# intel/neural-compressor

Hardware: AMD Instinct MI355X
Metric: llama2_7b_gptq_int4_g128_quantize_wall_clock (lower is better)
Workload: dtype bf16

## Files before the change

neural_compressor_amd/csrc/gptq.hip:

```cpp
#include <math.h>

#include <algorithm>
#include <type_traits>

#include "common.hpp"
#include "gptq_common.hpp"

namespace {

typedef __attribute__((ext_vector_type(16))) float f32x16;

template <int DT>
__global__ void gptq_prepare_weight_kernel(const void* __restrict__ w, float* __restrict__ out,
                                           const uint8_t* __restrict__ dead, int64_t N, int64_t K) {
  const int64_t total = N * K;
  for (int64_t i = blockIdx.x * (int64_t)blockDim.x + threadIdx.x; i < total;
       i += (int64_t)gridDim.x * blockDim.x) {
    const int64_t k = i % K;
    out[i] = (dead && dead[k]) ? 0.f : load_as_f32<DT>(w, i);
  }
}
template <int DT>
__global__ __launch_bounds__(256) void gptq_prepare_weight_vec_kernel(const void* __restrict__ w, float* __restrict__ out,
                                                                      const uint8_t* __restrict__ dead, int64_t N, int64_t K) {
  const int64_t k8 = K >> 3, total = N * k8;
  for (int64_t i = blockIdx.x * (int64_t)blockDim.x + threadIdx.x; i < total; i += (int64_t)gridDim.x * blockDim.x) {
    const int64_t n = i / k8, c = (i - n * k8) << 3, base = n * K + c;
    float v[8];
    if constexpr (DT == INC_F32) {
      const float4 a = reinterpret_cast<const float4*>(static_cast<const float*>(w) + base)[0];
      const float4 b = reinterpret_cast<const float4*>(static_cast<const float*>(w) + base)[1];
      v[0] = a.x; v[1] = a.y; v[2] = a.z; v[3] = a.w; v[4] = b.x; v[5] = b.y; v[6] = b.z; v[7] = b.w;
    } else {
      const uint4 q = *reinterpret_cast<const uint4*>(static_cast<const uint16_t*>(w) + base);
      const uint32_t u[4] = {q.x, q.y, q.z, q.w};
#pragma unroll
      for (int e = 0; e < 4; ++e) {
        if constexpr (DT == INC_BF16) {
          v[2 * e] = bf16_bits_to_f32((uint16_t)(u[e] & 0xffffu));
          v[2 * e + 1] = bf16_bits_to_f32((uint16_t)(u[e] >> 16));
        } else {
          v[2 * e] = f16_bits_to_f32((uint16_t)(u[e] & 0xffffu));
          v[2 * e + 1] = f16_bits_to_f32((uint16_t)(u[e] >> 16));
        }
      }
    }
    if (dead) {
      const uint2 d = *reinterpret_cast<const uint2*>(dead + c);
#pragma unroll
      for (int e = 0; e < 8; ++e)
        if (((e < 4 ? d.x : d.y) >> (8 * (e & 3))) & 0xffu) v[e] = 0.f;
    }
    reinterpret_cast<float4*>(out + base)[0] = make_float4(v[0], v[1], v[2], v[3]);
    reinterpret_cast<float4*>(out + base)[1] = make_float4(v[4], v[5], v[6], v[7]);
  }
}

constexpr int QROWS = 64;
constexpr int QPITCH = QB + 1;

#pragma clang fp contract(off)
template <int QDT>
__global__ __launch_bounds__(64) void gptq_quant_block_kernel(
    const float* __restrict__ w, const float* __restrict__ Hinv, const float* __restrict__ scale,
    const float* __restrict__ zero, uint8_t* __restrict__ codes, void* __restrict__ q_out,
    float* __restrict__ err, int64_t N, int64_t K, int64_t G, int64_t i1, int count, int gs, float maxq) {
  extern __shared__ __attribute__((aligned(16))) char smem_raw[];
  float* hs = reinterpret_cast<float*>(smem_raw);
  float* stage = hs + QB * QB;
  uint8_t* cst = reinterpret_cast<uint8_t*>(stage + QROWS * QPITCH);
  constexpr int CP = QB + 4;
  const int lane = threadIdx.x;
  const int64_t n0 = (int64_t)blockIdx.x * QROWS;
  const int64_t row = n0 + lane;

  for (int idx = lane; idx < QB * QB; idx += 64) {
    const int r = idx >> 7, c = idx & 127;
    hs[idx] = (r < count && c < count) ? Hinv[(i1 + r) * K + i1 + c] : (r == c ? 1.f : 0.f);
  }
  for (int idx = lane; idx < QROWS * QB; idx += 64) {
    const int r = idx >> 7, c = idx & 127;
    stage[r * QPITCH + c] = (n0 + r < N && c < count) ? w[(n0 + r) * K + i1 + c] : 0.f;
  }
  __syncthreads();
  float wr[QB];
#pragma unroll
  for (int j = 0; j < QB; ++j) wr[j] = stage[lane * QPITCH + j];
  __syncthreads();

  const int64_t srow = (row < N ? row : N - 1) * G;
  int g = gs > 0 ? (int)(i1 / gs) : 0;
  int nb = gs > 0 ? (int)(((int64_t)(g + 1)) * gs - i1) : (1 << 30);
  float s = scale[srow + g], z = zero[srow + g];
#pragma unroll
  for (int i = 0; i < QB; ++i) {
    if (i < count) {
      if (i == nb) {
        ++g;
        nb += gs;
        s = scale[srow + g];
        z = zero[srow + g];
      }
      const float d = hs[i * QB + i];
      const float x = wr[i];
      float t = rintf(x / s) + z;
      t = fminf(fmaxf(t, 0.f), maxq);
      const float q = s * (t - z);
      const float e = (x - q) / d;
      cst[lane * CP + i] = (uint8_t)t;
      stage[lane * QPITCH + i] = e;
      wr[i] = q;
#pragma unroll
      for (int j = i + 1; j < QB; ++j) {
        const float p = e * hs[i * QB + j];
        wr[j] = wr[j] - p;
      }
    } else {
      stage[lane * QPITCH + i] = 0.f;
      cst[lane * CP + i] = 0;
    }
  }
  __syncthreads();
  for (int idx = lane; idx < QROWS * QB; idx += 64) {
    const int r = idx >> 7, c = idx & 127;
    if (n0 + r < N) err[(n0 + r) * QB + c] = stage[r * QPITCH + c];
  }
  __syncthreads();
#pragma unroll
  for (int j = 0; j < QB; ++j) stage[lane * QPITCH + j] = wr[j];
  __syncthreads();
  for (int idx = lane; idx < QROWS * QB; idx += 64) {
    const int r = idx >> 7, c = idx & 127;
    if (n0 + r < N && c < count) {
      const int64_t o = (n0 + r) * K + i1 + c;
      if (q_out) store_from_f32<QDT>(q_out, o, stage[r * QPITCH + c]);
      if (codes) codes[o] = cst[r * CP + c];
    }
  }
}
#pragma clang fp contract(fast)

constexpr int Q4R = 16;
constexpr int Q4W = 4;
template <int I, int END, typename F>
__device__ __forceinline__ void static_for(F&& f) {
  if constexpr (I < END) {
    f(std::integral_constant<int, I>{});
    static_for<I + 1, END>(f);
  }
}
__device__ __forceinline__ float quad_bcast(float v, int src) {
  const int x = __float_as_int(v);
  int y;
  switch (src) {
    case 0: y = __builtin_amdgcn_mov_dpp(x, 0x00, 0xf, 0xf, true); break;
    case 1: y = __builtin_amdgcn_mov_dpp(x, 0x55, 0xf, 0xf, true); break;
    case 2: y = __builtin_amdgcn_mov_dpp(x, 0xAA, 0xf, 0xf, true); break;
    default: y = __builtin_amdgcn_mov_dpp(x, 0xFF, 0xf, 0xf, true); break;
  }
  return __int_as_float(y);
}
#pragma clang fp contract(off)
template <int QDT, int GPB, bool PARAMS = false, int WPW = 4>
__global__ __launch_bounds__(64 * WPW) void gptq_quant_block_q4_kernel(
    const float* __restrict__ w, const float* __restrict__ Hinv, float* __restrict__ scale,
    float* __restrict__ zero, uint8_t* __restrict__ codes, void* __restrict__ q_out,
    float* __restrict__ err, int64_t N, int64_t K, int64_t G, int64_t i1, int64_t g0, float maxq, int sym_flag) {
  extern __shared__ __attribute__((aligned(16))) char smem_raw[];
  float* hs = reinterpret_cast<float*>(smem_raw);
  __builtin_amdgcn_s_setprio(3);
  const int lane = threadIdx.x & 63, r = lane >> 2, q = lane & 3;
  const int wave = __builtin_amdgcn_readfirstlane((int)(threadIdx.x >> 6));
  const int64_t n0 = ((int64_t)blockIdx.x * WPW + wave) * Q4R;
  const int64_t row = n0 + r, rowc = row < N ? row : N - 1;

  {
    const uint32_t lds0 = (uint32_t)(uintptr_t)smem_raw;
    const float* hb = Hinv + i1 * K + i1;
    const uint32_t v0 = (uint32_t)(((lane >> 5) * K + 4 * (lane & 31)) * 4);
    const uint32_t step = (uint32_t)(2 * K * 4);
#pragma unroll
    for (int jj = 0; jj < 16 / WPW; ++jj) {
      const int j = jj * WPW + wave;
      lds_dma_4x1k(hb, lds0 + j * 4096, v0 + (4 * j) * step, v0 + (4 * j + 1) * step, v0 + (4 * j + 2) * step, v0 + (4 * j + 3) * step);
    }
  }
  float wr[32], ev[32];
  uint32_t cw[8];
#pragma unroll
  for (int c = 0; c < 32; ++c) {
    wr[c] = w[rowc * K + i1 + 4 * c + q];
    ev[c] = 0.f;
  }
#pragma unroll
  for (int c = 0; c < 8; ++c) cw[c] = 0u;
  float sg[GPB], zg[GPB];
  if constexpr (!PARAMS) {
#pragma unroll
    for (int g = 0; g < GPB; ++g) {
      sg[g] = scale[rowc * G + g0 + g];
      zg[g] = zero[rowc * G + g0 + g];
    }
  }
  asm volatile("s_waitcnt vmcnt(0)" ::: "memory");
  if constexpr (PARAMS) {
#pragma unroll
    for (int g = 0; g < GPB; ++g) {
      float vmax = -INFINITY, vmin = INFINITY;
#pragma unroll
      for (int c = g * (32 / GPB); c < (g + 1) * (32 / GPB); ++c) {
        vmax = fmaxf(vmax, wr[c]);
        vmin = fminf(vmin, wr[c]);
      }
      vmax = fmaxf(vmax, __shfl_xor(vmax, 1, 64));
      vmin = fminf(vmin, __shfl_xor(vmin, 1, 64));
      vmax = fmaxf(vmax, __shfl_xor(vmax, 2, 64));
      vmin = fminf(vmin, __shfl_xor(vmin, 2, 64));
      float xmin = fminf(vmin, 0.f), xmax = fmaxf(vmax, 0.f);
      if (sym_flag) {
        xmax = fmaxf(fabsf(xmin), xmax);
        if (xmin < 0.f) xmin = -xmax;
      }
      if (xmin == 0.f && xmax == 0.f) { xmin = -1.f; xmax = 1.f; }
      const float sv = (xmax - xmin) / maxq;
      const float zv = sym_flag ? (maxq + 1.f) * 0.5f : rintf(-xmin / sv);
      sg[g] = sv;
      zg[g] = zv;
      if (q == 0 && row < N) {
        scale[row * G + g0 + g] = sv;
        zero[row * G + g0 + g] = zv;
      }
    }
  }
  __syncthreads();

  float ha[33], hb2[33];
  auto fetch_row = [&](auto ic, float (&h)[33]) {
    constexpr int i = decltype(ic)::value;
    if constexpr (i < QB) {
#pragma unroll
      for (int c = i >> 2; c < 32; ++c) h[c] = hs[i * QB + 4 * c + q];
      h[32] = hs[i * QB + i];
    }
  };
  auto step = [&](auto ic, float (&h)[33]) {
    constexpr int i = decltype(ic)::value;
    constexpr int qo = i & 3, ci = i >> 2, g = i / (QB / GPB);
    const float s = sg[g], z = zg[g];
    const float x = quad_bcast(wr[ci], qo);
    float t = rintf(x / s) + z;
    t = fminf(fmaxf(t, 0.f), maxq);
    const float qv = s * (t - z);
    const float e = (x - qv) / h[32];
    const bool own = q == qo;
#pragma unroll
    for (int c = ci; c < 32; ++c) {
      const float pr = e * h[c];
      wr[c] = wr[c] - pr;
    }
    wr[ci] = own ? qv : wr[ci];
    ev[ci] = own ? e : ev[ci];
    cw[ci >> 2] = own ? (cw[ci >> 2] | ((uint32_t)t << (8 * (ci & 3)))) : cw[ci >> 2];
    asm volatile("" : "+v"(wr[ci]), "+v"(ev[ci]), "+v"(cw[ci >> 2]));
  };
  fetch_row(std::integral_constant<int, 0>{}, ha);
  static_for<0, QB / 2>([&](auto pc) {
    constexpr int p = decltype(pc)::value;
    fetch_row(std::integral_constant<int, 2 * p + 1>{}, hb2);
    step(std::integral_constant<int, 2 * p>{}, ha);
    fetch_row(std::integral_constant<int, 2 * p + 2>{}, ha);
    step(std::integral_constant<int, 2 * p + 1>{}, hb2);
  });
  __syncthreads();
  float* st = reinterpret_cast<float*>(smem_raw + wave * (Q4R * QB * 5));
#pragma unroll
  for (int c = 0; c < 32; ++c) st[r * QB + 4 * c + q] = ev[c];
  __syncthreads();
  for (int idx = lane; idx < Q4R * QB / 4; idx += 64) {
    const int rr = idx >> 5, c4 = (idx & 31) * 4;
    if (n0 + rr < N) *reinterpret_cast<float4*>(err + (n0 + rr) * QB + c4) = *reinterpret_cast<const float4*>(st + rr * QB + c4);
  }
  __syncthreads();
#pragma unroll
  for (int c = 0; c < 32; ++c) st[r * QB + 4 * c + q] = wr[c];
  uint8_t* cst = reinterpret_cast<uint8_t*>(st + Q4R * QB);
#pragma unroll
  for (int c = 0; c < 32; ++c) cst[r * QB + 4 * c + q] = (uint8_t)((cw[c >> 2] >> (8 * (c & 3))) & 0xffu);
  __syncthreads();
  for (int idx = lane; idx < Q4R * QB; idx += 64) {
    const int rr = idx >> 7, c = idx & 127;
    if (n0 + rr < N) {
      const int64_t o = (n0 + rr) * K + i1 + c;
      if (q_out) store_from_f32<QDT>(q_out, o, st[rr * QB + c]);
      if (codes) codes[o] = cst[rr * QB + c];
    }
  }
}
#pragma clang fp contract(fast)

constexpr int LT = 128;
constexpr int LAP = LT + 1;
__global__ __launch_bounds__(256) void gptq_lazy_update_kernel(float* __restrict__ w,
                                                               const float* __restrict__ Hinv,
                                                               const float* __restrict__ err, int64_t N,
                                                               int64_t K, int64_t i1, int count) {
  extern __shared__ __attribute__((aligned(16))) char smem_raw[];
  float* As = reinterpret_cast<float*>(smem_raw);
  float* Bs = As + LT * LAP;
  const int64_t i2 = i1 + count;
  const int64_t c0 = i2 + (int64_t)blockIdx.x * LT, r0 = (int64_t)blockIdx.y * LT;
  const int tid = threadIdx.x, lane = tid & 63, wave = tid >> 6;
  const int wr = wave >> 1, wc = wave & 1;
  for (int idx = tid; idx < LT * QB; idx += 256) {
    const int r = idx >> 7, k = idx & 127;
    As[r * LAP + k] = (r0 + r < N && k < count) ? err[(r0 + r) * QB + k] : 0.f;
  }
  for (int idx = tid; idx < QB * LT; idx += 256) {
    const int k = idx >> 7, c = idx & 127;
    Bs[idx] = (k < count && c0 + c < K) ? Hinv[(i1 + k) * K + c0 + c] : 0.f;
  }
  __syncthreads();
  f32x16 acc[2][2];
#pragma unroll
  for (int a = 0; a < 2; ++a)
#pragma unroll
    for (int b = 0; b < 2; ++b)
#pragma unroll
      for (int r = 0; r < 16; ++r) acc[a][b][r] = 0.f;
#pragma unroll 4
  for (int s = 0; s < QB / 2; ++s) {
    const int k = 2 * s + (lane >> 5);
    float a[2], b[2];
#pragma unroll
    for (int m = 0; m < 2; ++m) {
      a[m] = As[(wr * 64 + m * 32 + (lane & 31)) * LAP + k];
      b[m] = Bs[k * LT + wc * 64 + m * 32 + (lane & 31)];
    }
#pragma unroll
    for (int m = 0; m < 2; ++m)
#pragma unroll
      for (int n = 0; n < 2; ++n)
        acc[m][n] = __builtin_amdgcn_mfma_f32_32x32x2f32(a[m], b[n], acc[m][n], 0, 0, 0);
  }
#pragma unroll
  for (int m = 0; m < 2; ++m)
#pragma unroll
    for (int n = 0; n < 2; ++n) {
      const int64_t col = c0 + wc * 64 + n * 32 + (lane & 31);
#pragma unroll
      for (int r = 0; r < 16; ++r) {
        const int64_t row = r0 + wr * 64 + m * 32 + (r & 3) + 8 * (r >> 2) + 4 * (lane >> 5);
        if (row < N && col < K) {
          float* p = w + row * K + col;
          *p = *p - acc[m][n][r];
        }
      }
    }
}

#ifdef INC_KBENCH
#include "../../tools/kbench_gptq_2.inc"
#include "../../tools/kbench_gptq_3.inc"
#endif

template <bool PARAMS>
int launch_quant_block_q4(const float* w, const float* Hinv, float* scale, float* zero, uint8_t* codes, void* q_out, int q_dtype, float* err,
                          int64_t N, int64_t K, int64_t G, int64_t i1, int64_t g0, int gpb, float maxq, int sym, hipStream_t s) {
  const size_t smem4 = (size_t)QB * QB * 4;
  static std::atomic<uint64_t> attr_set{0};
  if (inc_attr_needed(attr_set)) {
    auto lds = [&](auto... kernel) { ((void)hipFuncSetAttribute((const void*)kernel, hipFuncAttributeMaxDynamicSharedMemorySize, (int)smem4), ...); };
    lds(gptq_quant_block_q4_kernel<INC_F32, 1, PARAMS>, gptq_quant_block_q4_kernel<INC_F32, 2, PARAMS>, gptq_quant_block_q4_kernel<INC_F32, 4, PARAMS>);
    lds(gptq_quant_block_q4_kernel<INC_F16, 1, PARAMS>, gptq_quant_block_q4_kernel<INC_F16, 2, PARAMS>, gptq_quant_block_q4_kernel<INC_F16, 4, PARAMS>);
    lds(gptq_quant_block_q4_kernel<INC_BF16, 1, PARAMS>, gptq_quant_block_q4_kernel<INC_BF16, 2, PARAMS>, gptq_quant_block_q4_kernel<INC_BF16, 4, PARAMS>);
    inc_attr_done(attr_set);
  }
  const unsigned blocks4 = (unsigned)ceil_div64(N, Q4R * Q4W);
  auto launch = [&](auto kernel) { kernel<<<blocks4, 64 * Q4W, smem4, s>>>(w, Hinv, scale, zero, codes, q_out, err, N, K, G, i1, g0, maxq, sym); };
  INC_DISPATCH_DTYPE(q_dtype, DT, {
    if (gpb == 1) launch(gptq_quant_block_q4_kernel<DT, 1, PARAMS>);
    else if (gpb == 2) launch(gptq_quant_block_q4_kernel<DT, 2, PARAMS>);
    else launch(gptq_quant_block_q4_kernel<DT, 4, PARAMS>);
  })
  INC_LAUNCH_RETURN();
}

bool lazy_update_range(float* w, const float* Hinv, const float* err, int64_t N, int64_t K, int64_t i1, int count, int64_t c_begin,
                       int64_t c_end, bool exclusive, hipStream_t s) {
  if (!lazy_block_ok(K, i1, count)) return false;
#ifdef INC_KBENCH
  if (lazy_update_lab_launch(w, Hinv, err, N, K, i1, c_begin, c_end, exclusive, s)) return true;
#endif
  inc_launch_lazy_update_v3(w, Hinv, err, N, K, i1, c_begin, c_end, exclusive, s);
  return true;
}

}

extern "C" {

int inc_gptq_prepare_weight(const void* w, int wdtype, float* out, const uint8_t* dead, int64_t N,
                            int64_t K, inc_stream_t stream) {
  INC_CHECK_ARG(w && out && N > 0 && K > 0);
  const bool vec = (K % 8) == 0 && ((reinterpret_cast<uintptr_t>(w) | reinterpret_cast<uintptr_t>(out)) & 15) == 0 &&
                   (!dead || (reinterpret_cast<uintptr_t>(dead) & 7) == 0);
  int64_t blocks = ceil_div64(vec ? N * (K / 8) : N * K, 256);
  if (blocks > 8192) blocks = 8192;
  INC_DISPATCH_DTYPE(wdtype, DT, {
    if (vec) gptq_prepare_weight_vec_kernel<DT><<<(unsigned)blocks, 256, 0, inc_s(stream)>>>(w, out, dead, N, K);
    else gptq_prepare_weight_kernel<DT><<<(unsigned)blocks, 256, 0, inc_s(stream)>>>(w, out, dead, N, K);
  })
  INC_LAUNCH_RETURN();
}

int inc_gptq_quant_block(const float* w, const float* Hinv, const float* scale, const float* zero,
                         uint8_t* codes, void* q_out, int q_dtype, float* err, int64_t N, int64_t K,
                         int64_t G, int64_t i1, int count, int group_size, int bits,
                         inc_stream_t stream) {
  INC_CHECK_ARG(w && Hinv && scale && zero && err && N > 0 && K > 0 && G > 0);
  INC_CHECK_ARG(i1 >= 0 && count > 0 && count <= QB && i1 + count <= K && bits >= 1 && bits <= 8);
  const float maxq = (float)((1 << bits) - 1);
  hipStream_t s = inc_s(stream);
  const int gpb = groups_per_block(group_size, true);
  if (gpb && chain_block_ok(K, i1, count) && !inc_force_small_tiles())
    return launch_quant_block_q4<false>(w, Hinv, const_cast<float*>(scale), const_cast<float*>(zero), codes, q_out, q_dtype, err, N, K, G, i1,
                                        group_size > 0 ? i1 / group_size : 0, gpb, maxq, 0, s);
  const size_t smem = (size_t)QB * QB * 4 + (size_t)QROWS * QPITCH * 4 + (size_t)QROWS * (QB + 4);
  static std::atomic<uint64_t> attr_set{0};
  if (inc_attr_needed(attr_set)) {
    (void)hipFuncSetAttribute((const void*)gptq_quant_block_kernel<INC_F32>, hipFuncAttributeMaxDynamicSharedMemorySize, (int)smem);
    (void)hipFuncSetAttribute((const void*)gptq_quant_block_kernel<INC_F16>, hipFuncAttributeMaxDynamicSharedMemorySize, (int)smem);
    (void)hipFuncSetAttribute((const void*)gptq_quant_block_kernel<INC_BF16>, hipFuncAttributeMaxDynamicSharedMemorySize, (int)smem);
    inc_attr_done(attr_set);
  }
  INC_DISPATCH_DTYPE(q_dtype, DT, {
    gptq_quant_block_kernel<DT><<<(unsigned)ceil_div64(N, QROWS), 64, smem, s>>>(w, Hinv, scale, zero, codes, q_out, err, N, K, G, i1, count, group_size, maxq);
  })
  INC_LAUNCH_RETURN();
}

int inc_gptq_quant_block_params(const float* w, const float* Hinv, float* scale, float* zero, uint8_t* codes, void* q_out,
                                int q_dtype, float* err, int64_t N, int64_t K, int64_t G, int64_t i1, int count, int group_size,
                                int bits, int sym, inc_stream_t stream) {
  INC_CHECK_ARG(w && Hinv && scale && zero && err && N > 0 && K > 0 && G > 0);
  INC_CHECK_ARG(i1 >= 0 && count > 0 && count <= QB && i1 + count <= K && bits >= 1 && bits <= 8);
  const int gpb = groups_per_block(group_size, false);
  if (!(gpb && chain_block_ok(K, i1, count))) return INC_ERR_UNSUPPORTED;
  const int64_t g0 = i1 / group_size;
  INC_CHECK_ARG(g0 + gpb <= G);
  return launch_quant_block_q4<true>(w, Hinv, scale, zero, codes, q_out, q_dtype, err, N, K, G, i1, g0, gpb, (float)((1 << bits) - 1), sym,
                                     inc_s(stream));
}

int inc_gptq_lazy_update(float* w, const float* Hinv, const float* err, int64_t N, int64_t K,
                         int64_t i1, int count, inc_stream_t stream) {
  INC_CHECK_ARG(w && Hinv && err && N > 0 && K > 0 && i1 >= 0 && count > 0 && count <= QB);
  const int64_t i2 = i1 + count;
  if (i2 >= K) return INC_OK;
  if (!inc_force_small_tiles() && lazy_update_range(w, Hinv, err, N, K, i1, count, i2, K, true, inc_s(stream))) INC_LAUNCH_RETURN();
  const size_t smem = (size_t)LT * LAP * 4 + (size_t)QB * LT * 4;
  static std::atomic<uint64_t> attr_set{0};
  if (inc_attr_needed(attr_set)) {
    (void)hipFuncSetAttribute((const void*)gptq_lazy_update_kernel, hipFuncAttributeMaxDynamicSharedMemorySize, (int)smem);
    inc_attr_done(attr_set);
  }
  dim3 grid((unsigned)ceil_div64(K - i2, LT), (unsigned)ceil_div64(N, LT));
  gptq_lazy_update_kernel<<<grid, 256, smem, inc_s(stream)>>>(w, Hinv, err, N, K, i1, count);
  INC_LAUNCH_RETURN();
}

int inc_gptq_lazy_update_cols(float* w, const float* Hinv, const float* err, int64_t N, int64_t K, int64_t i1, int count,
                              int64_t col_begin, int64_t col_end, inc_stream_t stream) {
  INC_CHECK_ARG(w && Hinv && err && N > 0 && K > 0 && i1 >= 0 && count > 0 && count <= QB);
  const int64_t i2 = i1 + count;
  INC_CHECK_ARG(col_begin >= i2 && col_end <= K && col_begin <= col_end && ((col_begin - i2) % L2T) == 0 &&
                (col_end == K || ((col_end - col_begin) % L2T) == 0));
  if (col_begin == col_end) return INC_OK;
  if (!lazy_update_range(w, Hinv, err, N, K, i1, count, col_begin, col_end, false, inc_s(stream))) return INC_ERR_UNSUPPORTED;
  INC_LAUNCH_RETURN();
}


int inc_gptq_quantize_layer(float* w, const float* Hinv, float* scale, float* zero, int64_t G, const float* loop_scale,
                            const float* loop_zero, int64_t loop_G, uint8_t* codes, void* q_out, int q_dtype, float* err_ws,
                            int64_t N, int64_t K, int group_size, int kernel_group_size, int block_size, int bits, int sym, int flags,
                            inc_stream_t stream, inc_stream_t aux_stream) {
  INC_CHECK_ARG(w && Hinv && scale && zero && err_ws && N > 0 && K > 0 && G > 0 && bits >= 1 && bits <= 8 && group_size > 0);
  const bool dynamic_groups = (flags & INC_GPTQ_DYNAMIC_GROUPS) != 0, mse = (flags & INC_GPTQ_MSE) != 0;
  const bool own_tables = loop_scale == nullptr || loop_scale == scale;
  if (own_tables) { loop_scale = scale; loop_zero = zero; loop_G = G; }
  INC_CHECK_ARG(loop_zero && loop_G > 0);
  const int64_t blocksize = block_size > 0 ? block_size : K;
  hipStream_t main = inc_s(stream), side = inc_s(aux_stream);
  const bool lookahead = aux_stream != nullptr && (flags & INC_GPTQ_NO_LOOKAHEAD) == 0 && K % QB == 0 && blocksize % QB == 0 && K >= 3 * QB;
  const bool fuse_params = (flags & INC_GPTQ_NO_FUSED_PARAMS) == 0 && dynamic_groups && !mse && blocksize == QB &&
                           groups_per_block(group_size, false) != 0 && K % QB == 0 && own_tables && chain_block_ok(K, 0, QB);
  float* errs[2] = {err_ws, err_ws + N * QB};
  hipEvent_t ready = nullptr, rest_done = nullptr;
  bool rest_pending = false;
  int rc = INC_OK;
#define INC_TRY(call)                  \
  {                                    \
    const int r_ = (call);             \
    if (r_ != INC_OK) { rc = r_; goto done; } \
  }
  if (lookahead) {
    if (hipEventCreateWithFlags(&ready, hipEventDisableTiming) != hipSuccess || hipEventCreateWithFlags(&rest_done, hipEventDisableTiming) != hipSuccess) {
      rc = INC_ERR_LAUNCH;
      goto done;
    }
    (void)hipEventRecord(ready, main);
    (void)hipStreamWaitEvent(side, ready, 0);
  }
  {
    int blk = 0;
    for (int64_t i1 = 0; i1 < K; ++blk) {
      const int64_t ref_end = std::min((i1 / blocksize + 1) * blocksize, K);
      const int count = (int)std::min<int64_t>(QB, ref_end - i1);
      if (dynamic_groups && i1 % blocksize == 0 && !fuse_params) {
        const int64_t g_first = (i1 + group_size - 1) / group_size, g_last = (ref_end - 1) / group_size;
        if (g_last >= g_first) {
          if (lookahead && rest_pending && (g_last + 1) * group_size > i1 + QB) (void)hipStreamWaitEvent(main, rest_done, 0);
          if (mse) INC_TRY(inc_gptq_find_params_mse(w, N, K, g_first * group_size, group_size, (int)(g_last - g_first + 1), bits, sym, 100, 0.8f, 2.4f, scale, zero, G, g_first, stream))
          else INC_TRY(inc_gptq_find_params(w, N, K, g_first * group_size, group_size, (int)(g_last - g_first + 1), bits, sym, scale, zero, G, g_first, stream))
        }
      }
      float* e = errs[lookahead ? (blk & 1) : 0];
      if (fuse_params) INC_TRY(inc_gptq_quant_block_params(w, Hinv, scale, zero, codes, q_out, q_dtype, e, N, K, G, i1, count, group_size, bits, sym, stream))
      else INC_TRY(inc_gptq_quant_block(w, Hinv, loop_scale, loop_zero, codes, q_out, q_dtype, e, N, K, loop_G, i1, count, kernel_group_size, bits, stream))
      const int64_t i2 = i1 + count;
      if (!lookahead) {
        INC_TRY(inc_gptq_lazy_update(w, Hinv, e, N, K, i1, count, stream))
      } else if (i2 < K) {
        const int64_t nxt_end = std::min<int64_t>(i2 + QB, K);
        if (nxt_end < K) (void)hipEventRecord(ready, main);
        if (rest_pending) (void)hipStreamWaitEvent(main, rest_done, 0);
        INC_TRY(inc_gptq_lazy_update_cols(w, Hinv, e, N, K, i1, count, i2, nxt_end, stream))
        if (nxt_end < K) {
          (void)hipStreamWaitEvent(side, ready, 0);
          INC_TRY(inc_gptq_lazy_update_cols(w, Hinv, e, N, K, i1, count, nxt_end, K, aux_stream))
          (void)hipEventRecord(rest_done, side);
          rest_pending = true;
        }
      }
      i1 = i2;
    }
  }
  if (lookahead && rest_pending) (void)hipStreamWaitEvent(main, rest_done, 0);
done:
#undef INC_TRY
  if (ready) (void)hipEventDestroy(ready);
  if (rest_done) (void)hipEventDestroy(rest_done);
  return rc;
}

#ifdef INC_KBENCH
int64_t inc_debug_lazy_x3_bytes(int64_t N, int64_t K) { return lazyx3_planes_bytes(K, K) + 2 * lazyx3_planes_bytes(N, 128); }
int inc_debug_lazy_x3_prepare(const float* Hinv, int64_t N, int64_t K, void* planes, inc_stream_t stream) {
  LazyX3State& g = g_lazyx3;
  if (!planes) { g = LazyX3State(); return INC_OK; }
  uint16_t* hp = static_cast<uint16_t*>(planes);
  lazyx3_split(Hinv, K, K, K, true, hp, &g.hinv_plane, &g.hinv_rp, inc_s(stream));
  g.hinv_planes = hp;
  g.err_planes = reinterpret_cast<uint16_t*>(static_cast<char*>(planes) + lazyx3_planes_bytes(K, K));
  INC_LAUNCH_RETURN();
}
#endif

}
```

neural_compressor_amd/csrc/gptq_common.hpp:

```cpp
#pragma once
#include <hip/hip_runtime.h>

constexpr int QB = 128;
constexpr int L2T = 128;

void inc_launch_lazy_update_v3(float* w, const float* Hinv, const float* err, int64_t N, int64_t K, int64_t i1, int64_t c_begin,
                               int64_t c_end, bool exclusive, hipStream_t s);

static inline bool block_range_ok(int64_t K, int count) { return count == QB && (K % 4) == 0 && K * (int64_t)(QB + 1) * 4 < ((int64_t)1 << 32); }
static inline bool chain_block_ok(int64_t K, int64_t i1, int count) { return (i1 % QB) == 0 && block_range_ok(K, count); }
static inline bool lazy_block_ok(int64_t K, int64_t i1, int count) { return (i1 % 4) == 0 && block_range_ok(K, count); }

static inline int groups_per_block(int group_size, bool allow_ungrouped) {
  if (allow_ungrouped ? (group_size <= 0 || (group_size % QB) == 0) : group_size == QB) return 1;
  return group_size == 64 ? 2 : group_size == 32 ? 4 : 0;
}

enum IncGptqLabFlag {
  LAB_HESSIAN_ROUND_LAUNCHES = 43,
  LAB_HESSIAN_NO_TAIL_SPLIT = 44,
  LAB_HESSIAN_REG_TRANSPOSE = 45,
  LAB_HESSIAN_STAGES_4X32 = 46,
  LAB_HESSIAN_NO_DMA = 47,
  LAB_HESSIAN_NO_MFMA = 48,
  LAB_HESSIAN_NO_DMA_NO_MFMA = 49,
  LAB_HESSIAN_SPREAD = 50,
  LAB_HESSIAN_SPREAD_4X32 = 51,
  LAB_HESSIAN_SPREAD_ROLL = 52,
  LAB_HESSIAN_ROLL = 53,
  LAB_HESSIAN_PRIO = 54,
  LAB_HESSIAN_SPREAD_ROLL_PRIO = 55,
  LAB_HESSIAN_ROLL_PRIO = 56,
  LAB_HESSIAN_PIPELINE = 57,
  LAB_HESSIAN_PIPELINE_PRIO = 58,
  LAB_HESSIAN_ROUND4 = 59,
  LAB_HESSIAN_PRODUCT_FORM = 60,
  LAB_LAZY_V2 = 86,
  LAB_LAZY_NO_MFMA = 87,
  LAB_LAZY_NO_LOADS = 88,
  LAB_LAZY_NO_STORES = 90,
  LAB_LAZY_X3 = 106,
  LAB_LAZY_V3_ONLY = 107,
  LAB_LAZY_STRIP_CAP_4 = 108,
  LAB_LAZY_STRIP_CAP_16 = 109,
  LAB_LAZY_SHORT_STRIPS = 110,
  LAB_CHOL_DIAG_V1 = 201,
};
```

neural_compressor_amd/csrc/gptq_lazy.hip:

```cpp
#include <algorithm>
#include <type_traits>

#include "common.hpp"
#include "gptq_common.hpp"

namespace {

typedef __attribute__((ext_vector_type(16))) float f32x16;

template <int CW>
__global__ __launch_bounds__(256, 2) void gptq_lazy_update_v3_kernel(float* __restrict__ w, const float* __restrict__ Hinv,
                                                                     const float* __restrict__ err, int64_t N, int64_t K,
                                                                     int64_t i1, int64_t c_begin) {
  constexpr int NF = CW / 32;
  constexpr uint32_t HS_OFF = CW == 128 ? 0u : 65536u;
  if constexpr (CW != 128) __builtin_amdgcn_s_setprio(2);
  extern __shared__ __attribute__((aligned(16))) char smem_raw[];
  const uint32_t lds0 = (uint32_t)(uintptr_t)smem_raw;
  const int tid = threadIdx.x, lane = tid & 63;
  const int wave = __builtin_amdgcn_readfirstlane(tid >> 6);
  const int64_t r0 = (int64_t)blockIdx.y * L2T + wave * 32;
  const int64_t c0 = c_begin + (int64_t)blockIdx.x * CW;
  const float* const hbase = Hinv + i1 * K;

  auto dma_hinv = [&]() {
    if constexpr (CW == 128) {
      int64_t col = c0 + 4 * (lane & 31);
      if (col > K - 4) col = K - 4;
      const uint32_t v = (uint32_t)(((wave * 32 + (lane >> 5)) * K + col) * 4);
      const uint32_t step = (uint32_t)(2 * K * 4);
      const uint32_t dst = __builtin_amdgcn_readfirstlane(lds0 + HS_OFF + wave * 16384);
#pragma unroll
      for (int q4 = 0; q4 < 4; ++q4)
        lds_dma_4x1k(hbase, dst + q4 * 4096, v + (4 * q4) * step, v + (4 * q4 + 1) * step, v + (4 * q4 + 2) * step, v + (4 * q4 + 3) * step);
    } else {
      int64_t col = c0 + 4 * (lane & 7);
      if (col > K - 4) col = K - 4;
      const uint32_t v = (uint32_t)(((wave * 32 + (lane >> 3)) * K + col) * 4);
      const uint32_t step = (uint32_t)(8 * K * 4);
      const uint32_t dst = __builtin_amdgcn_readfirstlane(lds0 + HS_OFF + wave * 4096);
      lds_dma_4x1k(hbase, dst, v, v + step, v + 2 * step, v + 3 * step);
    }
  };
  {
    const uint32_t dst = __builtin_amdgcn_readfirstlane(lds0 + wave * 16384);
    const int64_t rows_here = N - r0 < 32 ? N - r0 : 32;
    const float* ebase = err + (rows_here > 0 ? r0 : N - 1) * QB;
    uint32_t v[16];
#pragma unroll
    for (int j = 0; j < 16; ++j) {
      const int R = 2 * j + (lane >> 5);
      const int Rc = rows_here > 0 ? (R < rows_here ? R : (int)rows_here - 1) : 0;
      v[j] = (uint32_t)(Rc * (QB * 4)) + (uint32_t)(((lane & 31) ^ (R & 7)) * 16);
    }
#pragma unroll
    for (int q4 = 0; q4 < 4; ++q4) lds_dma_4x1k(ebase, dst + q4 * 4096, v[4 * q4], v[4 * q4 + 1], v[4 * q4 + 2], v[4 * q4 + 3]);
  }
  if constexpr (CW != 128) dma_hinv();
  float wt[NF][16];
#pragma unroll
  for (int nf = 0; nf < NF; ++nf) {
    int64_t col = c0 + nf * 32 + (lane & 31);
    if (col > K - 1) col = K - 1;
#pragma unroll
    for (int r = 0; r < 16; ++r) {
      int64_t row = r0 + (r & 3) + 8 * (r >> 2) + 4 * (lane >> 5);
      if (row > N - 1) row = N - 1;
      wt[nf][r] = w[row * K + col];
    }
  }
  f32x16 acc[NF];
#pragma unroll
  for (int nf = 0; nf < NF; ++nf)
#pragma unroll
    for (int r = 0; r < 16; ++r) acc[nf][r] = 0.f;
  if constexpr (CW == 128) asm volatile("s_waitcnt vmcnt(63)" ::: "memory");
  else asm volatile("s_waitcnt vmcnt(20)" ::: "memory");
  float a[64];
  {
    const int R = lane & 31;
    const char* eb = smem_raw + wave * 16384 + R * 512;
    const bool hi = (lane >> 5) != 0;
#pragma unroll
    for (int j = 0; j < 32; ++j) {
      const float4 v4 = *reinterpret_cast<const float4*>(eb + ((j ^ (R & 7)) * 16));
      a[2 * j] = hi ? v4.y : v4.x;
      a[2 * j + 1] = hi ? v4.w : v4.z;
    }
  }
  if constexpr (CW == 128) {
    asm volatile("s_waitcnt lgkmcnt(0)" ::: "memory");
    dma_hinv();
  }
  asm volatile("s_waitcnt vmcnt(0)" ::: "memory");
  __syncthreads();
  const float* hs = reinterpret_cast<const float*>(smem_raw + HS_OFF) + (lane >> 5) * CW + (lane & 31);
  constexpr int BS = NF == 4 ? 4 : 8;
#pragma unroll
  for (int g = 0; g < 64 / BS; ++g) {
    float b[BS * NF];
#pragma unroll
    for (int sb = 0; sb < BS; ++sb)
#pragma unroll
      for (int nf = 0; nf < NF; ++nf) b[sb * NF + nf] = hs[(2 * (BS * g + sb)) * CW + nf * 32];
#pragma unroll
    for (int sb = 0; sb < BS; ++sb)
#pragma unroll
      for (int nf = 0; nf < NF; ++nf) {
        acc[nf] = __builtin_amdgcn_mfma_f32_32x32x2f32(a[BS * g + sb], b[sb * NF + nf], acc[nf], 0, 0, 0);
      }
  }
  if (r0 + 32 <= N && c0 + CW <= K) {
#pragma unroll
    for (int nf = 0; nf < NF; ++nf) {
      float* wp = w + (r0 + 4 * (lane >> 5)) * K + c0 + nf * 32 + (lane & 31);
#pragma unroll
      for (int r = 0; r < 16; ++r) wp[((r & 3) + 8 * (r >> 2)) * K] = wt[nf][r] - acc[nf][r];
    }
  } else {
#pragma unroll
    for (int nf = 0; nf < NF; ++nf) {
      const int64_t col = c0 + nf * 32 + (lane & 31);
#pragma unroll
      for (int r = 0; r < 16; ++r) {
        const int64_t row = r0 + (r & 3) + 8 * (r >> 2) + 4 * (lane >> 5);
        if (row < N && col < K) w[row * K + col] = wt[nf][r] - acc[nf][r];
      }
    }
  }
}

#ifndef INC_LAZY_STRIP_TILES
#define INC_LAZY_STRIP_TILES 2048
#endif
#ifndef INC_LAZY_STRIP_CAP
#define INC_LAZY_STRIP_CAP 8
#endif
struct LazyLabOverrides {
  int ablation = 0;
  bool v3_everywhere = false;
  int64_t strip_cap = INC_LAZY_STRIP_CAP;
  bool never_one_round = false;
};

#ifdef INC_KBENCH
#include "../../tools/kbench_gptq_lazy_lab.inc"
#endif

constexpr int L4W = 32;

__global__ __launch_bounds__(256, 2) void gptq_lazy_update_v4_kernel(float* __restrict__ w, const float* __restrict__ Hinv,
                                                                     const float* __restrict__ err, int64_t N, int64_t K, int64_t i1,
                                                                     int64_t c_begin, int64_t c_end, int tiles_per_wg) {
  extern __shared__ __attribute__((aligned(16))) char smem_raw[];
  const uint32_t lds0 = (uint32_t)(uintptr_t)smem_raw;
  const int tid = threadIdx.x, lane = tid & 63;
  const int wave = __builtin_amdgcn_readfirstlane(tid >> 6);
  const int64_t r0 = (int64_t)blockIdx.y * L2T + wave * 32;
  const int64_t col0 = c_begin + (int64_t)blockIdx.x * tiles_per_wg * L4W;
  int tiles = (int)((c_end - col0 + L4W - 1) / L4W);
  if (tiles > tiles_per_wg) tiles = tiles_per_wg;
  const float* const hbase = Hinv + i1 * K;
  const int rows_here = (int)(N - r0 < 32 ? (N - r0 > 0 ? N - r0 : 0) : 32);
  const float* const wbase = w + (rows_here > 0 ? r0 : N - 1) * K;
  const uint32_t slice = __builtin_amdgcn_readfirstlane(lds0 + wave * 16384);
  const uint32_t h_step = (uint32_t)(8 * K * 4);
  const uint32_t h_row = (uint32_t)((wave * 32 + (lane >> 3)) * K * 4);
  uint32_t w_row[4];
#pragma unroll
  for (int q = 0; q < 4; ++q) {
    int R = 8 * q + (lane >> 3);
    R = rows_here > 0 ? (R < rows_here ? R : rows_here - 1) : 0;
    w_row[q] = (uint32_t)(R * K * 4);
  }
  auto request = [&](int64_t c0, int b) {
    int64_t col = c0 + 4 * (lane & 7);
    if (col > K - 4) col = K - 4;
    const uint32_t cb = (uint32_t)(col * 4);
    lds_dma_4x1k(hbase, slice + b * 4096, h_row + cb, h_row + h_step + cb, h_row + 2 * h_step + cb, h_row + 3 * h_step + cb);
    lds_dma_4x1k(wbase, slice + 8192 + b * 4096, w_row[0] + cb, w_row[1] + cb, w_row[2] + cb, w_row[3] + cb);
  };

  {
    const float* ebase = err + (rows_here > 0 ? r0 : N - 1) * QB;
    uint32_t v[16];
#pragma unroll
    for (int j = 0; j < 16; ++j) {
      const int R = 2 * j + (lane >> 5);
      const int Rc = rows_here > 0 ? (R < rows_here ? R : rows_here - 1) : 0;
      v[j] = (uint32_t)(Rc * (QB * 4)) + (uint32_t)(((lane & 31) ^ (R & 7)) * 16);
    }
#pragma unroll
    for (int q4 = 0; q4 < 4; ++q4) lds_dma_4x1k(ebase, slice + q4 * 4096, v[4 * q4], v[4 * q4 + 1], v[4 * q4 + 2], v[4 * q4 + 3]);
  }
  asm volatile("s_waitcnt vmcnt(0)" ::: "memory");
  float a[64];
  {
    const int R = lane & 31;
    const char* eb = smem_raw + wave * 16384 + R * 512;
    const bool hi = (lane >> 5) != 0;
#pragma unroll
    for (int j = 0; j < 32; ++j) {
      const float4 v4 = *reinterpret_cast<const float4*>(eb + ((j ^ (R & 7)) * 16));
      a[2 * j] = hi ? v4.y : v4.x;
      a[2 * j + 1] = hi ? v4.w : v4.z;
    }
  }
  asm volatile("s_waitcnt lgkmcnt(0)" ::: "memory");
  request(col0, 0);

  const char* const hs0 = smem_raw + lane * 4;
  const char* const ws0 = smem_raw + wave * 16384 + 8192 + (lane >> 5) * 512 + (lane & 31) * 4;
  float* const wp0 = w + (r0 + 4 * (lane >> 5)) * K + (lane & 31);
  bool counted = false;
  for (int t = 0; t < tiles; ++t) {
    const int b = t & 1;
    const int64_t c0 = col0 + (int64_t)t * L4W;
    if (counted) asm volatile("s_waitcnt vmcnt(16)" ::: "memory");
    else asm volatile("s_waitcnt vmcnt(0)" ::: "memory");
    __syncthreads();
    if (t + 1 < tiles) request(c0 + L4W, b ^ 1);
    f32x16 acc;
#pragma unroll
    for (int r = 0; r < 16; ++r) acc[r] = 0.f;
    const char* hs = hs0 + b * 4096;
    constexpr int BS = 8;
    float bq[2][BS];
#pragma unroll
    for (int sb = 0; sb < BS; ++sb) bq[0][sb] = *reinterpret_cast<const float*>(hs + ((2 * sb) >> 5) * 16384 + ((2 * sb) & 31) * 128);
#pragma unroll
    for (int g = 0; g < 64 / BS; ++g) {
      if (g + 1 < 64 / BS) {
#pragma unroll
        for (int sb = 0; sb < BS; ++sb) {
          const int s2 = 2 * (BS * (g + 1) + sb);
          bq[(g + 1) & 1][sb] = *reinterpret_cast<const float*>(hs + (s2 >> 5) * 16384 + (s2 & 31) * 128);
        }
      }
      __builtin_amdgcn_sched_barrier(0);
#pragma unroll
      for (int sb = 0; sb < BS; ++sb) acc = __builtin_amdgcn_mfma_f32_32x32x2f32(a[BS * g + sb], bq[g & 1][sb], acc, 0, 0, 0);
      __builtin_amdgcn_sched_barrier(0);
    }
    const char* ws = ws0 + b * 4096;
    float wt[16];
#pragma unroll
    for (int r = 0; r < 16; ++r) wt[r] = *reinterpret_cast<const float*>(ws + ((r & 3) + 8 * (r >> 2)) * 128);
    counted = r0 + 32 <= N && c0 + L4W <= K;
    if (counted) {
      float* wp = wp0 + c0;
#pragma unroll
      for (int r = 0; r < 16; ++r) wp[((r & 3) + 8 * (r >> 2)) * K] = wt[r] - acc[r];
    } else {
      const int64_t col = c0 + (lane & 31);
#pragma unroll
      for (int r = 0; r < 16; ++r) {
        const int64_t row = r0 + (r & 3) + 8 * (r >> 2) + 4 * (lane >> 5);
        if (row < N && col < K) w[row * K + col] = wt[r] - acc[r];
      }
    }
    asm volatile("" ::: "memory");
  }
}

int64_t lazy_strip_plan(int64_t row_tiles, int64_t nt4, bool exclusive, int64_t cap, bool force_short) {
  constexpr int64_t SLOTS = 512, CUS = 256, STARTUP = 3;
  const int64_t chunks_one = SLOTS / row_tiles > 0 ? SLOTS / row_tiles : 1;
  int64_t tpw_one = ceil_div64(nt4, chunks_one);
  if (tpw_one < 4) tpw_one = 4;
  const int64_t cost_one = ceil_div64(ceil_div64(nt4, tpw_one) * row_tiles, CUS) * (tpw_one + STARTUP);
  int64_t tpw_short = nt4 / ceil_div64(SLOTS, row_tiles);
  if (tpw_short > cap) tpw_short = cap;
  if (tpw_short < 4) tpw_short = 4;
  const int64_t cost_short = ceil_div64(ceil_div64(nt4, tpw_short) * row_tiles, CUS) * (2 * tpw_short + STARTUP) / 2;
  const bool one_round = !force_short && exclusive && ceil_div64(nt4, tpw_one) * row_tiles <= SLOTS && cost_one <= cost_short;
  return one_round ? tpw_one : tpw_short;
}

}

void inc_launch_lazy_update_v3(float* w, const float* Hinv, const float* err, int64_t N, int64_t K, int64_t i1, int64_t c_begin,
                               int64_t c_end, bool exclusive, hipStream_t s) {
  static std::atomic<uint64_t> attr_set{0};
  if (inc_attr_needed(attr_set)) {
    (void)hipFuncSetAttribute((const void*)gptq_lazy_update_v3_kernel<128>, hipFuncAttributeMaxDynamicSharedMemorySize, 65536);
    (void)hipFuncSetAttribute((const void*)gptq_lazy_update_v3_kernel<32>, hipFuncAttributeMaxDynamicSharedMemorySize, 65536 + L2T * 32 * 4);
    inc_attr_done(attr_set);
  }
  const int64_t row_tiles = ceil_div64(N, L2T);
  const int64_t col_tiles = ceil_div64(c_end - c_begin, L2T);
#ifdef INC_KBENCH
  const LazyLabOverrides lab = lazy_lab_overrides();
  if (lab.ablation) return lazy_lab_ablation_launch(lab.ablation, w, Hinv, err, N, K, i1, c_begin, col_tiles, row_tiles, s);
#else
  constexpr LazyLabOverrides lab;
#endif
  const int64_t nt4 = ceil_div64(c_end - c_begin, L4W);
  if (row_tiles * nt4 >= (int64_t)INC_LAZY_STRIP_TILES && !lab.v3_everywhere) {
    static std::atomic<uint64_t> attr4_set{0};
    if (inc_attr_needed(attr4_set)) {
      (void)hipFuncSetAttribute((const void*)gptq_lazy_update_v4_kernel, hipFuncAttributeMaxDynamicSharedMemorySize, 65536);
      inc_attr_done(attr4_set);
    }
    const int64_t tpw = lazy_strip_plan(row_tiles, nt4, exclusive, lab.strip_cap, lab.never_one_round);
    gptq_lazy_update_v4_kernel<<<dim3((unsigned)ceil_div64(nt4, tpw), (unsigned)row_tiles), 256, 65536, s>>>(w, Hinv, err, N, K, i1, c_begin, c_end, (int)tpw);
    return;
  }
  if (row_tiles * col_tiles <= 128)
    gptq_lazy_update_v3_kernel<32><<<dim3((unsigned)ceil_div64(c_end - c_begin, 32), (unsigned)row_tiles), 256, 65536 + L2T * 32 * 4, s>>>(w, Hinv, err, N, K, i1, c_begin);
  else
    gptq_lazy_update_v3_kernel<128><<<dim3((unsigned)col_tiles, (unsigned)row_tiles), 256, 65536, s>>>(w, Hinv, err, N, K, i1, c_begin);
}
```

Measured before the change: 7.336.

## Halve quant-block LDS via two-stage Hinv loading; add small lazy-update kernel

```diff
diff --git a/neural_compressor_amd/csrc/gptq.hip b/neural_compressor_amd/csrc/gptq.hip
--- a/neural_compressor_amd/csrc/gptq.hip
+++ b/neural_compressor_amd/csrc/gptq.hip
@@ -161,6 +161,7 @@
   return __int_as_float(y);
 }
 #pragma clang fp contract(off)
+constexpr int QH = QB / 2;
 template <int QDT, int GPB, bool PARAMS = false, int WPW = 4>
 __global__ __launch_bounds__(64 * WPW) void gptq_quant_block_q4_kernel(
     const float* __restrict__ w, const float* __restrict__ Hinv, float* __restrict__ scale,
@@ -168,23 +169,26 @@
     float* __restrict__ err, int64_t N, int64_t K, int64_t G, int64_t i1, int64_t g0, float maxq, int sym_flag) {
   extern __shared__ __attribute__((aligned(16))) char smem_raw[];
   float* hs = reinterpret_cast<float*>(smem_raw);
+  static_assert(WPW == 4, "the two stages of the Hinv1 tile are shared out over four waves");
   __builtin_amdgcn_s_setprio(3);
   const int lane = threadIdx.x & 63, r = lane >> 2, q = lane & 3;
   const int wave = __builtin_amdgcn_readfirstlane((int)(threadIdx.x >> 6));
   const int64_t n0 = ((int64_t)blockIdx.x * WPW + wave) * Q4R;
   const int64_t row = n0 + r, rowc = row < N ? row : N - 1;
 
+  const uint32_t lds0 = (uint32_t)(uintptr_t)smem_raw;
+  const float* const hb = Hinv + i1 * K + i1;
   {
-    const uint32_t lds0 = (uint32_t)(uintptr_t)smem_raw;
-    const float* hb = Hinv + i1 * K + i1;
     const uint32_t v0 = (uint32_t)(((lane >> 5) * K + 4 * (lane & 31)) * 4);
     const uint32_t step = (uint32_t)(2 * K * 4);
 #pragma unroll
-    for (int jj = 0; jj < 16 / WPW; ++jj) {
+    for (int jj = 0; jj < 8 / WPW; ++jj) {
       const int j = jj * WPW + wave;
       lds_dma_4x1k(hb, lds0 + j * 4096, v0 + (4 * j) * step, v0 + (4 * j + 1) * step, v0 + (4 * j + 2) * step, v0 + (4 * j + 3) * step);
     }
   }
+  const uint32_t v2 = (uint32_t)(((QH + 16 * wave + (lane >> 4)) * K + QH + 4 * (lane & 15)) * 4);
+  const uint32_t step2 = (uint32_t)(4 * K * 4);
   float wr[32], ev[32];
   uint32_t cw[8];
 #pragma unroll
@@ -237,10 +241,14 @@
   float ha[33], hb2[33];
   auto fetch_row = [&](auto ic, float (&h)[33]) {
     constexpr int i = decltype(ic)::value;
-    if constexpr (i < QB) {
+    if constexpr (i < QH) {
 #pragma unroll
       for (int c = i >> 2; c < 32; ++c) h[c] = hs[i * QB + 4 * c + q];
       h[32] = hs[i * QB + i];
+    } else if constexpr (i < QB) {
+#pragma unroll
+      for (int c = i >> 2; c < 32; ++c) h[c] = hs[(i - QH) * QH + 4 * c + q - QH];
+      h[32] = hs[(i - QH) * QH + i - QH];
     }
   };
   auto step = [&](auto ic, float (&h)[33]) {
@@ -266,13 +274,21 @@
   fetch_row(std::integral_constant<int, 0>{}, ha);
   static_for<0, QB / 2>([&](auto pc) {
     constexpr int p = decltype(pc)::value;
+    if constexpr (2 * p == QH / 2) {
+      __syncthreads();
+      lds_dma_4x1k(hb, lds0 + wave * 4096, v2, v2 + step2, v2 + 2 * step2, v2 + 3 * step2);
+    }
     fetch_row(std::integral_constant<int, 2 * p + 1>{}, hb2);
     step(std::integral_constant<int, 2 * p>{}, ha);
+    if constexpr (2 * p + 2 == QH) {
+      asm volatile("s_waitcnt vmcnt(0)" ::: "memory");
+      __syncthreads();
+    }
     fetch_row(std::integral_constant<int, 2 * p + 2>{}, ha);
     step(std::integral_constant<int, 2 * p + 1>{}, hb2);
   });
   __syncthreads();
-  float* st = reinterpret_cast<float*>(smem_raw + wave * (Q4R * QB * 5));
+  float* st = reinterpret_cast<float*>(smem_raw + wave * (Q4R * QB * 4));
 #pragma unroll
   for (int c = 0; c < 32; ++c) st[r * QB + 4 * c + q] = ev[c];
   __syncthreads();
@@ -283,20 +299,30 @@
   __syncthreads();
 #pragma unroll
   for (int c = 0; c < 32; ++c) st[r * QB + 4 * c + q] = wr[c];
-  uint8_t* cst = reinterpret_cast<uint8_t*>(st + Q4R * QB);
+  __syncthreads();
+  if (q_out) {
+    for (int idx = lane; idx < Q4R * QB; idx += 64) {
+      const int rr = idx >> 7, c = idx & 127;
+      if (n0 + rr < N) store_from_f32<QDT>(q_out, (n0 + rr) * K + i1 + c, st[rr * QB + c]);
+    }
+  }
+  __syncthreads();
+  uint8_t* cst = reinterpret_cast<uint8_t*>(st);
 #pragma unroll
   for (int c = 0; c < 32; ++c) cst[r * QB + 4 * c + q] = (uint8_t)((cw[c >> 2] >> (8 * (c & 3))) & 0xffu);
   __syncthreads();
-  for (int idx = lane; idx < Q4R * QB; idx += 64) {
-    const int rr = idx >> 7, c = idx & 127;
-    if (n0 + rr < N) {
-      const int64_t o = (n0 + rr) * K + i1 + c;
-      if (q_out) store_from_f32<QDT>(q_out, o, st[rr * QB + c]);
-      if (codes) codes[o] = cst[rr * QB + c];
+  if (codes) {
+    for (int idx = lane; idx < Q4R * QB; idx += 64) {
+      const int rr = idx >> 7, c = idx & 127;
+      if (n0 + rr < N) codes[(n0 + rr) * K + i1 + c] = cst[rr * QB + c];
     }
   }
 }
 #pragma clang fp contract(fast)
+
+#ifdef INC_KBENCH
+#include "../../tools/kbench_gptq_chain64.inc"
+#endif
 
 constexpr int LT = 128;
 constexpr int LAP = LT + 1;
@@ -366,16 +392,23 @@
 template <bool PARAMS>
 int launch_quant_block_q4(const float* w, const float* Hinv, float* scale, float* zero, uint8_t* codes, void* q_out, int q_dtype, float* err,
                           int64_t N, int64_t K, int64_t G, int64_t i1, int64_t g0, int gpb, float maxq, int sym, hipStream_t s) {
-  const size_t smem4 = (size_t)QB * QB * 4;
-  static std::atomic<uint64_t> attr_set{0};
-  if (inc_attr_needed(attr_set)) {
-    auto lds = [&](auto... kernel) { ((void)hipFuncSetAttribute((const void*)kernel, hipFuncAttributeMaxDynamicSharedMemorySize, (int)smem4), ...); };
-    lds(gptq_quant_block_q4_kernel<INC_F32, 1, PARAMS>, gptq_quant_block_q4_kernel<INC_F32, 2, PARAMS>, gptq_quant_block_q4_kernel<INC_F32, 4, PARAMS>);
-    lds(gptq_quant_block_q4_kernel<INC_F16, 1, PARAMS>, gptq_quant_block_q4_kernel<INC_F16, 2, PARAMS>, gptq_quant_block_q4_kernel<INC_F16, 4, PARAMS>);
-    lds(gptq_quant_block_q4_kernel<INC_BF16, 1, PARAMS>, gptq_quant_block_q4_kernel<INC_BF16, 2, PARAMS>, gptq_quant_block_q4_kernel<INC_BF16, 4, PARAMS>);
-    inc_attr_done(attr_set);
-  }
   const unsigned blocks4 = (unsigned)ceil_div64(N, Q4R * Q4W);
+#ifdef INC_KBENCH
+  if (inc_small_tiles_flag(-1) == LAB_COLLOOP_LDS64) {
+    const size_t smem64 = (size_t)QB * QB * 4;
+    auto launch64 = [&](auto kernel) {
+      (void)hipFuncSetAttribute((const void*)kernel, hipFuncAttributeMaxDynamicSharedMemorySize, (int)smem64);
+      kernel<<<blocks4, 64 * Q4W, smem64, s>>>(w, Hinv, scale, zero, codes, q_out, err, N, K, G, i1, g0, maxq, sym);
+    };
+    INC_DISPATCH_DTYPE(q_dtype, DT, {
+      if (gpb == 1) launch64(gptq_quant_block_q4_lds64_kernel<DT, 1, PARAMS>);
+      else if (gpb == 2) launch64(gptq_quant_block_q4_lds64_kernel<DT, 2, PARAMS>);
+      else launch64(gptq_quant_block_q4_lds64_kernel<DT, 4, PARAMS>);
+    })
+    INC_LAUNCH_RETURN();
+  }
+#endif
+  const size_t smem4 = (size_t)QH * QB * 4;
   auto launch = [&](auto kernel) { kernel<<<blocks4, 64 * Q4W, smem4, s>>>(w, Hinv, scale, zero, codes, q_out, err, N, K, G, i1, g0, maxq, sym); };
   INC_DISPATCH_DTYPE(q_dtype, DT, {
     if (gpb == 1) launch(gptq_quant_block_q4_kernel<DT, 1, PARAMS>);
diff --git a/neural_compressor_amd/csrc/gptq_common.hpp b/neural_compressor_amd/csrc/gptq_common.hpp
--- a/neural_compressor_amd/csrc/gptq_common.hpp
+++ b/neural_compressor_amd/csrc/gptq_common.hpp
@@ -44,5 +44,6 @@
   LAB_LAZY_STRIP_CAP_4 = 108,
   LAB_LAZY_STRIP_CAP_16 = 109,
   LAB_LAZY_SHORT_STRIPS = 110,
+  LAB_COLLOOP_LDS64 = 111,
   LAB_CHOL_DIAG_V1 = 201,
 };
diff --git a/neural_compressor_amd/csrc/gptq_lazy.hip b/neural_compressor_amd/csrc/gptq_lazy.hip
--- a/neural_compressor_amd/csrc/gptq_lazy.hip
+++ b/neural_compressor_amd/csrc/gptq_lazy.hip
@@ -8,13 +8,11 @@
 
 typedef __attribute__((ext_vector_type(16))) float f32x16;
 
-template <int CW>
 __global__ __launch_bounds__(256, 2) void gptq_lazy_update_v3_kernel(float* __restrict__ w, const float* __restrict__ Hinv,
                                                                      const float* __restrict__ err, int64_t N, int64_t K,
                                                                      int64_t i1, int64_t c_begin) {
-  constexpr int NF = CW / 32;
-  constexpr uint32_t HS_OFF = CW == 128 ? 0u : 65536u;
-  if constexpr (CW != 128) __builtin_amdgcn_s_setprio(2);
+  constexpr int CW = 128, NF = CW / 32;
+  constexpr uint32_t HS_OFF = 0u;
   extern __shared__ __attribute__((aligned(16))) char smem_raw[];
   const uint32_t lds0 = (uint32_t)(uintptr_t)smem_raw;
   const int tid = threadIdx.x, lane = tid & 63;
@@ -24,23 +22,14 @@
   const float* const hbase = Hinv + i1 * K;
 
   auto dma_hinv = [&]() {
-    if constexpr (CW == 128) {
-      int64_t col = c0 + 4 * (lane & 31);
-      if (col > K - 4) col = K - 4;
-      const uint32_t v = (uint32_t)(((wave * 32 + (lane >> 5)) * K + col) * 4);
-      const uint32_t step = (uint32_t)(2 * K * 4);
-      const uint32_t dst = __builtin_amdgcn_readfirstlane(lds0 + HS_OFF + wave * 16384);
-#pragma unroll
-      for (int q4 = 0; q4 < 4; ++q4)
-        lds_dma_4x1k(hbase, dst + q4 * 4096, v + (4 * q4) * step, v + (4 * q4 + 1) * step, v + (4 * q4 + 2) * step, v + (4 * q4 + 3) * step);
-    } else {
-      int64_t col = c0 + 4 * (lane & 7);
-      if (col > K - 4) col = K - 4;
-      const uint32_t v = (uint32_t)(((wave * 32 + (lane >> 3)) * K + col) * 4);
-      const uint32_t step = (uint32_t)(8 * K * 4);
-      const uint32_t dst = __builtin_amdgcn_readfirstlane(lds0 + HS_OFF + wave * 4096);
-      lds_dma_4x1k(hbase, dst, v, v + step, v + 2 * step, v + 3 * step);
-    }
+    int64_t col = c0 + 4 * (lane & 31);
+    if (col > K - 4) col = K - 4;
+    const uint32_t v = (uint32_t)(((wave * 32 + (lane >> 5)) * K + col) * 4);
+    const uint32_t step = (uint32_t)(2 * K * 4);
+    const uint32_t dst = __builtin_amdgcn_readfirstlane(lds0 + HS_OFF + wave * 16384);
+#pragma unroll
+    for (int q4 = 0; q4 < 4; ++q4)
+      lds_dma_4x1k(hbase, dst + q4 * 4096, v + (4 * q4) * step, v + (4 * q4 + 1) * step, v + (4 * q4 + 2) * step, v + (4 * q4 + 3) * step);
   };
   {
     const uint32_t dst = __builtin_amdgcn_readfirstlane(lds0 + wave * 16384);
@@ -56,7 +45,6 @@
 #pragma unroll
     for (int q4 = 0; q4 < 4; ++q4) lds_dma_4x1k(ebase, dst + q4 * 4096, v[4 * q4], v[4 * q4 + 1], v[4 * q4 + 2], v[4 * q4 + 3]);
   }
-  if constexpr (CW != 128) dma_hinv();
   float wt[NF][16];
 #pragma unroll
   for (int nf = 0; nf < NF; ++nf) {
@@ -74,8 +62,7 @@
   for (int nf = 0; nf < NF; ++nf)
 #pragma unroll
     for (int r = 0; r < 16; ++r) acc[nf][r] = 0.f;
-  if constexpr (CW == 128) asm volatile("s_waitcnt vmcnt(63)" ::: "memory");
-  else asm volatile("s_waitcnt vmcnt(20)" ::: "memory");
+  asm volatile("s_waitcnt vmcnt(63)" ::: "memory");
   float a[64];
   {
     const int R = lane & 31;
@@ -88,14 +75,12 @@
       a[2 * j + 1] = hi ? v4.w : v4.z;
     }
   }
-  if constexpr (CW == 128) {
-    asm volatile("s_waitcnt lgkmcnt(0)" ::: "memory");
-    dma_hinv();
-  }
+  asm volatile("s_waitcnt lgkmcnt(0)" ::: "memory");
+  dma_hinv();
   asm volatile("s_waitcnt vmcnt(0)" ::: "memory");
   __syncthreads();
   const float* hs = reinterpret_cast<const float*>(smem_raw + HS_OFF) + (lane >> 5) * CW + (lane & 31);
-  constexpr int BS = NF == 4 ? 4 : 8;
+  constexpr int BS = 4;
 #pragma unroll
   for (int g = 0; g < 64 / BS; ++g) {
     float b[BS * NF];
@@ -126,6 +111,98 @@
         const int64_t row = r0 + (r & 3) + 8 * (r >> 2) + 4 * (lane >> 5);
         if (row < N && col < K) w[row * K + col] = wt[nf][r] - acc[nf][r];
       }
+    }
+  }
+}
+
+constexpr int LNR = 32;
+__global__ __launch_bounds__(256, 2) void gptq_lazy_update_next_kernel(float* __restrict__ w, const float* __restrict__ Hinv,
+                                                                       const float* __restrict__ err, int64_t N, int64_t K, int64_t i1,
+                                                                       int64_t c_begin) {
+  __builtin_amdgcn_s_setprio(2);
+  extern __shared__ __attribute__((aligned(16))) char smem_raw[];
+  const uint32_t lds0 = (uint32_t)(uintptr_t)smem_raw;
+  const int tid = threadIdx.x, lane = tid & 63;
+  const int wave = __builtin_amdgcn_readfirstlane(tid >> 6);
+  const int64_t r0 = (int64_t)blockIdx.y * LNR;
+  const int64_t c0 = c_begin + (int64_t)blockIdx.x * L2T + wave * 32;
+  {
+    const int rows_here = (int)(N - r0 < LNR ? N - r0 : LNR);
+    uint32_t v[4];
+#pragma unroll
+    for (int j = 0; j < 4; ++j) {
+      const int R = 8 * wave + 2 * j + (lane >> 5);
+      const int Rc = R < rows_here ? R : rows_here - 1;
+      v[j] = (uint32_t)(Rc * (QB * 4)) + (uint32_t)(((lane & 31) ^ (R & 7)) * 16);
+    }
+    lds_dma_4x1k(err + r0 * QB, __builtin_amdgcn_readfirstlane(lds0 + wave * 4096), v[0], v[1], v[2], v[3]);
+  }
+  int64_t colc = c0 + (lane & 31);
+  if (colc > K - 1) colc = K - 1;
+  const int hi4 = 4 * (lane >> 5);
+  const uint32_t hoff = (uint32_t)(((lane >> 5) * K + colc) * 4);
+  constexpr int BS = 16;
+  float bq[2][BS];
+  auto load_b = [&](int g, float (&b)[BS]) {
+    uint32_t o = hoff;
+    asm volatile("" : "+v"(o));
+#pragma unroll
+    for (int sb = 0; sb < BS; ++sb)
+      b[sb] = *reinterpret_cast<const float*>(reinterpret_cast<const char*>(Hinv + (i1 + 2 * (BS * g + sb)) * K) + o);
+  };
+  load_b(0, bq[0]);
+  load_b(1, bq[1]);
+  const int last_row = (int)(N - r0 < LNR ? N - r0 : LNR) - 1;
+  const char* const wrows = reinterpret_cast<const char*>(w + r0 * K);
+  float wt[16];
+  auto load_w = [&]() {
+    int h = hi4;
+    asm volatile("" : "+v"(h));
+#pragma unroll
+    for (int r = 0; r < 16; ++r) {
+      int row = (r & 3) + 8 * (r >> 2) + h;
+      if (row > last_row) row = last_row;
+      wt[r] = *reinterpret_cast<const float*>(wrows + ((uint32_t)row * (uint32_t)K + (uint32_t)colc) * 4u);
+    }
+  };
+  asm volatile("s_waitcnt vmcnt(0)" ::: "memory");
+  __syncthreads();
+  float a[64];
+  {
+    const int R = lane & 31;
+    const char* eb = smem_raw + R * 512;
+    const bool hi = (lane >> 5) != 0;
+#pragma unroll
+    for (int j = 0; j < 32; ++j) {
+      if ((j & 3) == 0) __builtin_amdgcn_sched_barrier(0);
+      const float4 v4 = *reinterpret_cast<const float4*>(eb + ((j ^ (R & 7)) * 16));
+      a[2 * j] = hi ? v4.y : v4.x;
+      a[2 * j + 1] = hi ? v4.w : v4.z;
+    }
+  }
+  f32x16 acc;
+#pragma unroll
+  for (int r = 0; r < 16; ++r) acc[r] = 0.f;
+#pragma unroll
+  for (int g = 0; g < 64 / BS; ++g) {
+    __builtin_amdgcn_sched_barrier(0);
+#pragma unroll
+    for (int sb = 0; sb < BS; ++sb) acc = __builtin_amdgcn_mfma_f32_32x32x2f32(a[BS * g + sb], bq[g & 1][sb], acc, 0, 0, 0);
+    __builtin_amdgcn_sched_barrier(0);
+    if (g + 2 < 64 / BS) load_b(g + 2, bq[g & 1]);
+    if (g == 0) load_w();
+  }
+  if (r0 + LNR <= N && c0 + 32 <= K) {
+    const uint32_t woff = (uint32_t)((hi4 * K + colc) * 4);
+#pragma unroll
+    for (int r = 0; r < 16; ++r)
+      *reinterpret_cast<float*>(reinterpret_cast<char*>(w + (r0 + (r & 3) + 8 * (r >> 2)) * K) + woff) = wt[r] - acc[r];
+  } else {
+    const int64_t col = c0 + (lane & 31);
+#pragma unroll
+    for (int r = 0; r < 16; ++r) {
+      const int64_t row = r0 + (r & 3) + 8 * (r >> 2) + hi4;
+      if (row < N && col < K) w[row * K + col] = wt[r] - acc[r];
     }
   }
 }
@@ -141,6 +218,7 @@
   bool v3_everywhere = false;
   int64_t strip_cap = INC_LAZY_STRIP_CAP;
   bool never_one_round = false;
+  bool next_lds80 = false;
 };
 
 #ifdef INC_KBENCH
@@ -283,8 +361,7 @@
                                int64_t c_end, bool exclusive, hipStream_t s) {
   static std::atomic<uint64_t> attr_set{0};
   if (inc_attr_needed(attr_set)) {
-    (void)hipFuncSetAttribute((const void*)gptq_lazy_update_v3_kernel<128>, hipFuncAttributeMaxDynamicSharedMemorySize, 65536);
-    (void)hipFuncSetAttribute((const void*)gptq_lazy_update_v3_kernel<32>, hipFuncAttributeMaxDynamicSharedMemorySize, 65536 + L2T * 32 * 4);
+    (void)hipFuncSetAttribute((const void*)gptq_lazy_update_v3_kernel, hipFuncAttributeMaxDynamicSharedMemorySize, 65536);
     inc_attr_done(attr_set);
   }
   const int64_t row_tiles = ceil_div64(N, L2T);
@@ -306,8 +383,12 @@
     gptq_lazy_update_v4_kernel<<<dim3((unsigned)ceil_div64(nt4, tpw), (unsigned)row_tiles), 256, 65536, s>>>(w, Hinv, err, N, K, i1, c_begin, c_end, (int)tpw);
     return;
   }
-  if (row_tiles * col_tiles <= 128)
-    gptq_lazy_update_v3_kernel<32><<<dim3((unsigned)ceil_div64(c_end - c_begin, 32), (unsigned)row_tiles), 256, 65536 + L2T * 32 * 4, s>>>(w, Hinv, err, N, K, i1, c_begin);
-  else
-    gptq_lazy_update_v3_kernel<128><<<dim3((unsigned)col_tiles, (unsigned)row_tiles), 256, 65536, s>>>(w, Hinv, err, N, K, i1, c_begin);
-}
+  if (row_tiles * col_tiles <= 128) {
+#ifdef INC_KBENCH
+    if (lab.next_lds80) return lazy_lab_quarter_launch(w, Hinv, err, N, K, i1, c_begin, c_end, row_tiles, s);
+#endif
+    gptq_lazy_update_next_kernel<<<dim3((unsigned)col_tiles, (unsigned)ceil_div64(N, LNR)), 256, LNR * QB * 4, s>>>(w, Hinv, err, N, K, i1, c_begin);
+  } else {
+    gptq_lazy_update_v3_kernel<<<dim3((unsigned)col_tiles, (unsigned)row_tiles), 256, 65536, s>>>(w, Hinv, err, N, K, i1, c_begin);
+  }
+}
```

Measured after the change: 7.337. Within noise of the previous version (+0.0%).
